# FengDushuo/BBBP-Multi-Modal-Deep-Ensemble-Framework

Measured on AMD Instinct MI355X. Metric: molecules/sec fwd+bwd (3-branch ensemble, B=512), higher is better.
Workload: dtype f32; 1 GPU; MixedInputModel F=167 (MACCS) + 3x128x128 image, 6-layer encoder + 2-stage CNN + fusion + BN head; forward + MSE + backward + fused AdamW, train mode (dropout 0.1); global_batch=512, per_gpu_batch=512, parallelism=dp1, input=device-resident

## Files before the change

bbbp-multi-modal-deep-ensemble-framework_amd/csrc/gemm.hip:

```cpp
#include "common.h"
#include "bbbp_hip.h"
#include <mutex>
#include <type_traits>
#include <unordered_map>

#define TRY_RC(expr) do { int _rc = (expr); if (_rc) return _rc; } while (0)

typedef float f32x4u __attribute__((ext_vector_type(4), aligned(4)));
typedef float f32x2u __attribute__((ext_vector_type(2), aligned(4)));

namespace {

constexpr int bk_of(int tile) { return tile == 64 ? 16 : 32; }

struct GemmParams {
    const float* A; const float* B; float* C;
    const float* bias; const float* R;
    int M, N, K;
    int lda, ldb, ldc, ldr;
    long sA, sB, sC, sR;
    float alpha;
    int act;
    int splits, kchunk;
    float* slab;
// ... 944 lines not shown
    constexpr bool A_KMAJ = (LAYOUT == 2), B_KMAJ = (LAYOUT != 0);
#ifndef BBBP_DIRECT_DEPTH
#define BBBP_DIRECT_DEPTH 4
#endif
    constexpr int D = BBBP_DIRECT_DEPTH;
    const int lane = threadIdx.x & 63, wave = threadIdx.x >> 6;
    const int ks = wave % p.ks, sp = wave / p.ks;
    const int wm = sp / p.wsn, wn = sp % p.wsn;
    DirectOperand<TM, A_KMAJ> opa;
    DirectOperand<TN, B_KMAJ> opb;
    opa.init(p.A + (long)batch * p.sA, p.lda, p.M, (blockIdx.y * p.wsm + wm) * 16 * TM, lane);
    opb.init(p.B + (long)batch * p.sB, p.ldb, p.N, (blockIdx.x * p.wsn + wn) * 16 * TN, lane);

    f32x4 acc[TM][TN];
#pragma unroll
    for (int i = 0; i < TM; ++i)
#pragma unroll
        for (int j = 0; j < TN; ++j) acc[i][j] = f32x4{0.f, 0.f, 0.f, 0.f};
    auto mfma_chunk = [&](const float (&a)[4][TM], const float (&b)[4][TN]) __attribute__((always_inline)) {
#pragma unroll
        for (int j = 0; j < 4; ++j)
#pragma unroll
            for (int um = 0; um < TM; ++um)
#pragma unroll
                for (int un = 0; un < TN; ++un)
                    acc[um][un] = __builtin_amdgcn_mfma_f32_16x16x4f32(a[j][um], b[j][un], acc[um][un], 0, 0, 0);
    };

    const int nch = (p.K + 15) / 16;
    bool has_ones = false;
    if constexpr (LAYOUT == 2) has_ones = p.asum != nullptr && opb.base <= p.N && p.N < opb.base + 16 * TN;
    const int nfast = (nch - 1 > ks) ? (nch - 1 - ks + p.ks - 1) / p.ks : 0;
    if (nfast > 0) {
        float ra[D][4][TM], rb[D][4][TN];
#pragma unroll
        for (int d = 0; d < D; ++d) {
            const int c = ks + min(d, nfast - 1) * p.ks;
            opa.fetch(c, ra[d]); opb.fetch(c, rb[d]);
        }
        for (int i0 = 0; i0 < nfast; i0 += D) {
#pragma unroll
            for (int d = 0; d < D; ++d) {
                if (i0 + d < nfast) {
                    if (has_ones) opb.ones(rb[d], 0, p.K);
                    mfma_chunk(ra[d], rb[d]);
                }
                const int c = ks + min(i0 + d + D, nfast - 1) * p.ks;
                opa.fetch(c, ra[d]); opb.fetch(c, rb[d]);
            }
        }
    }
    if (nch > 0 && (nch - 1) % p.ks == ks) {
        float ta[4][TM], tb[4][TN];
        opa.fetch_tail(nch - 1, p.K, ta); opb.fetch_tail(nch - 1, p.K, tb);
        if (has_ones) opb.ones(tb, nch - 1, p.K);
        mfma_chunk(ta, tb);
    }

    if (p.ks > 1) {
        float* mine = red + (long)wave * (TM * TN * 4 * 64) + lane;
        if (ks != 0) {
#pragma unroll
            for (int um = 0; um < TM; ++um)
#pragma unroll
                for (int un = 0; un < TN; ++un)
#pragma unroll
                    for (int r = 0; r < 4; ++r) mine[((um * TN + un) * 4 + r) * 64] = acc[um][un][r];
        }
        __syncthreads();
        if (ks != 0) return;
        for (int s = 1; s < p.ks; ++s) {
            const float* other = mine + (long)s * (TM * TN * 4 * 64);
#pragma unroll
            for (int um = 0; um < TM; ++um)
#pragma unroll
                for (int un = 0; un < TN; ++un)
#pragma unroll
                    for (int r = 0; r < 4; ++r) acc[um][un][r] += other[((um * TN + un) * 4 + r) * 64];
        }
    }

    float* C = p.C + (long)batch * p.sC;
    const float* R = p.R ? p.R + (long)batch * p.sR : nullptr;
    const int q = lane & 15, kq = lane >> 4;
#pragma unroll
    for (int un = 0; un < TN; ++un) {
        const int n = opb.index(un, q);
        const float bv = (p.bias && n < p.N) ? p.bias[n] : 0.f;
#pragma unroll
        for (int um = 0; um < TM; ++um)
#pragma unroll
            for (int r = 0; r < 4; ++r) {
                const int m = opa.index(um, 4 * kq + r);
                if constexpr (LAYOUT == 2) {
                    if (p.asum && n == p.N && m < p.M) p.asum[(long)batch * p.M + m] = acc[um][un][r];
                }
                if (m < p.M && n < p.N) {
                    float v = apply_act(p.alpha * acc[um][un][r] + bv, p.act);
                    if (p.drop_p > 0.f)
                        v *= dropout_scale(effective_seed(p.drop_seed, p.seed_base), ((uint64_t)batch * p.M + m) * p.N + n, p.drop_p, p.drop_inv_keep);
                    const float gsel = p.gate ? (p.gate[(long)batch * p.sG + (long)m * p.ldg + n] > 0.f ? p.gate_scale : 0.f) : 1.f;
                    if (!p.gate_after) v *= gsel;
                    if (R) v += R[(long)m * p.ldr + n];
                    if (p.gate_after) v *= gsel;
                    C[(long)m * p.ldc + n] = v;
                }
            }
    }
}

template <int LAYOUT, int TM, int TN>
__global__ __launch_bounds__(1024) void gemm_direct_kernel(DirectParams p) {
    BBBP_HIGH_PRIO();
    extern __shared__ float red[];
    gemm_direct_body<LAYOUT, TM, TN>(p, blockIdx.z, red);
}

struct LnFuse {
    const float* gamma; const float* beta;
    float* y; int ldy;
    float* mean; float* rstd;
    float eps;
};

__global__ __launch_bounds__(1024, 2) void gemm_direct_ln_kernel(DirectParams p, LnFuse f) {
    BBBP_HIGH_PRIO();
    __shared__ float part[2][16][16];
    constexpr int D = 4;
    const int lane = threadIdx.x & 63, wave = threadIdx.x >> 6, nw = blockDim.x >> 6;
    const int q = lane & 15, kq = lane >> 4;
    DirectOperand<1, false> opa, opb;
    opa.init(p.A, p.lda, p.M, blockIdx.y * 16, lane);
    opb.init(p.B, p.ldb, p.N, wave * 16, lane);
    f32x4 acc = {0.f, 0.f, 0.f, 0.f};
    auto mfma_chunk = [&](const float (&a)[4][1], const float (&b)[4][1]) __attribute__((always_inline)) {
#pragma unroll
        for (int j = 0; j < 4; ++j) acc = __builtin_amdgcn_mfma_f32_16x16x4f32(a[j][0], b[j][0], acc, 0, 0, 0);
    };
    const int nch = (p.K + 15) / 16;
    const int nfast = nch - 1;
    if (nfast > 0) {
        float ra[D][4][1], rb[D][4][1];
#pragma unroll
        for (int d = 0; d < D; ++d) { const int c = min(d, nfast - 1); opa.fetch(c, ra[d]); opb.fetch(c, rb[d]); }
        for (int i0 = 0; i0 < nfast; i0 += D) {
#pragma unroll
            for (int d = 0; d < D; ++d) {
                if (i0 + d < nfast) mfma_chunk(ra[d], rb[d]);
                const int c = min(i0 + d + D, nfast - 1);
                opa.fetch(c, ra[d]); opb.fetch(c, rb[d]);
            }
        }
    }
    if (nch > 0) {
        float ta[4][1], tb[4][1];
        opa.fetch_tail(nch - 1, p.K, ta); opb.fetch_tail(nch - 1, p.K, tb);
        mfma_chunk(ta, tb);
    }
    const int n = wave * 16 + q, m0 = blockIdx.y * 16 + 4 * kq;
    const bool coln = n < p.N;
    const float bv = (p.bias && coln) ? p.bias[n] : 0.f;
    const uint64_t seed = effective_seed(p.drop_seed, p.seed_base);
    float z[4], s[4];
#pragma unroll
    for (int r = 0; r < 4; ++r) {
        const int m = min(m0 + r, p.M - 1);
        float v = p.alpha * acc[r] + bv;
        if (p.drop_p > 0.f) v *= dropout_scale(seed, (uint64_t)m * p.N + min(n, p.N - 1), p.drop_p, p.drop_inv_keep);
        if (p.R && coln) v += p.R[(long)m * p.ldr + n];
        z[r] = coln ? v : 0.f;
        if (coln && m0 + r < p.M) p.C[(long)m * p.ldc + n] = v;
        s[r] = z[r];
    }
#pragma unroll
    for (int r = 0; r < 4; ++r) { s[r] += __shfl_xor(s[r], 1); s[r] += __shfl_xor(s[r], 2); s[r] += __shfl_xor(s[r], 4); s[r] += __shfl_xor(s[r], 8); }
    if (q == 0) {
#pragma unroll
        for (int r = 0; r < 4; ++r) part[0][wave][4 * kq + r] = s[r];
    }
    __syncthreads();
    float mean[4], d2[4];
#pragma unroll
    for (int r = 0; r < 4; ++r) {
        float t = 0.f;
        for (int w = 0; w < nw; ++w) t += part[0][w][4 * kq + r];
        mean[r] = t / p.N;
        const float d = coln ? z[r] - mean[r] : 0.f;
        d2[r] = d * d;
    }
#pragma unroll
    for (int r = 0; r < 4; ++r) { d2[r] += __shfl_xor(d2[r], 1); d2[r] += __shfl_xor(d2[r], 2); d2[r] += __shfl_xor(d2[r], 4); d2[r] += __shfl_xor(d2[r], 8); }
// ... 574 lines not shown
```

bbbp-multi-modal-deep-ensemble-framework_amd/csrc/rowops.hip:

```cpp
#include "common.h"
#include "bbbp_hip.h"
#include <stdlib.h>
#include <mutex>

namespace {

__device__ __forceinline__ float wave_sum(float v) {
#pragma unroll
    for (int o = 32; o > 0; o >>= 1) v += __shfl_xor(v, o);
    return v;
}
__device__ __forceinline__ float wave_max(float v) {
#pragma unroll
    for (int o = 32; o > 0; o >>= 1) v = fmaxf(v, __shfl_xor(v, o));
    return v;
}

__global__ __launch_bounds__(256) void layernorm_fwd_kernel(float* x, const float* r, float* y, const float* gamma,
                                                           const float* beta, float* mean_out, float* rstd_out,
                                                           int rows, int cols, float eps, float p, uint64_t seed_in, const unsigned long long* seed_base) {
    const uint64_t seed = effective_seed(seed_in, seed_base);
    BBBP_HIGH_PRIO();
    const int lane = threadIdx.x & 63;
    const int row = blockIdx.x * 4 + (threadIdx.x >> 6);
// ... 149 lines not shown
        if (q < nq) {
            const float4 v = make_float4(rs * (g[i].x - s1 - xh[i].x * s2), rs * (g[i].y - s1 - xh[i].y * s2),
                                         rs * (g[i].z - s1 - xh[i].z * s2), rs * (g[i].w - s1 - xh[i].w * s2));
            dzr[q] = v;
            if (dxr) {
                if (p > 0.f) {
                    const float4 k = dropout_scale4(seed, ((uint64_t)row * cols >> 2) + q, p, inv_keep);
                    dxr[q] = make_float4(v.x * k.x, v.y * k.y, v.z * k.z, v.w * k.w);
                } else {
                    dxr[q] = v;
                }
            }
        }
    }
}
inline int ln_wide_nv(int cols) {
    static const int on = bbbp_env_int("BBBP_LN_WIDE", 1);
    return (on && cols >= 1024 && cols <= 4096 && cols % 4 == 0) ? (cols + 1023) / 1024 : 0;
}

constexpr int CW = 16, RL = 32;
__global__ __launch_bounds__(512) void layernorm_param_grad_kernel(const float* dy, const float* z, const float* mean,
                                                                   const float* rstd, float* dgamma, float* dbeta,
                                                                   int rows, int cols) {
    BBBP_HIGH_PRIO();
    __shared__ float s1[RL][CW], s2[RL][CW];
    const int cl = threadIdx.x % CW, rl = threadIdx.x / CW;
    const int c = blockIdx.x * CW + cl;
    float a = 0.f, b = 0.f;
    if (c < cols)
        for (int r = rl; r < rows; r += RL) {
            float g = dy[(long)r * cols + c];
            a += g * (z[(long)r * cols + c] - mean[r]) * rstd[r];
            b += g;
        }
    s1[rl][cl] = a; s2[rl][cl] = b;
    __syncthreads();
    if (rl == 0 && c < cols) {
        float ta = 0.f, tb = 0.f;
#pragma unroll 8
        for (int i = 0; i < RL; ++i) { ta += s1[i][cl]; tb += s2[i][cl]; }
        dgamma[c] = ta; dbeta[c] = tb;
    }
}

__global__ __launch_bounds__(256) void softmax_fwd_kernel(float* x, float* pd, long rows, int cols, float p, uint64_t seed_in, const unsigned long long* seed_base) {
    const uint64_t seed = effective_seed(seed_in, seed_base);
    BBBP_HIGH_PRIO();
    const int lane = threadIdx.x & 63;
    const long row = (long)blockIdx.x * 4 + (threadIdx.x >> 6);
    if (row >= rows) return;
    float* xr = x + row * cols;
    float m = -INFINITY;
    for (int c = lane; c < cols; c += 64) m = fmaxf(m, xr[c]);
    m = wave_max(m);
    float s = 0.f;
    for (int c = lane; c < cols; c += 64) { float e = __expf(xr[c] - m); xr[c] = e; s += e; }
    const float inv = 1.f / wave_sum(s);
    const float inv_keep = p > 0.f ? 1.f / (1.f - p) : 1.f;
    for (int c = lane; c < cols; c += 64) {
        float v = xr[c] * inv;
        xr[c] = v;
        if (pd) pd[row * cols + c] = v * dropout_scale(seed, (uint64_t)row * cols + c, p, inv_keep);
    }
}

__global__ __launch_bounds__(256) void softmax_bwd_kernel(float* dpd, const float* prob, long rows, int cols, float p, uint64_t seed_in, const unsigned long long* seed_base) {
    const uint64_t seed = effective_seed(seed_in, seed_base);
    BBBP_HIGH_PRIO();
    const int lane = threadIdx.x & 63;
    const long row = (long)blockIdx.x * 4 + (threadIdx.x >> 6);
    if (row >= rows) return;
    float* dr = dpd + row * cols;
    const float* pr = prob + row * cols;
    const float inv_keep = p > 0.f ? 1.f / (1.f - p) : 1.f;
    float s = 0.f;
    for (int c = lane; c < cols; c += 64) {
        float d = dr[c];
        if (p > 0.f) { d *= dropout_scale(seed, (uint64_t)row * cols + c, p, inv_keep); dr[c] = d; }
        s += d * pr[c];
    }
    s = wave_sum(s);
    for (int c = lane; c < cols; c += 64) dr[c] = pr[c] * (dr[c] - s);
}

__global__ __launch_bounds__(256) void dropout_kernel(const float* x, float* y, long n, float p, uint64_t seed_in, const unsigned long long* seed_base) {
    const uint64_t seed = effective_seed(seed_in, seed_base);
    BBBP_HIGH_PRIO();
    const float inv_keep = 1.f / (1.f - p);
    for (long i = (long)blockIdx.x * 256 + threadIdx.x; i < n; i += (long)gridDim.x * 256)
        y[i] = x[i] * dropout_scale(seed, (uint64_t)i, p, inv_keep);
}

__global__ __launch_bounds__(1024) void batchnorm_fwd_kernel(const float* x, float* y, const float* gamma, const float* beta,
                                                            float* running_mean, float* running_var, float* save_mean,
                                                            float* save_rstd, int rows, int cols, float eps, float momentum,
                                                            int training) {
    BBBP_HIGH_PRIO();
    __shared__ float red[16][64];
    __shared__ float smean[64], srstd[64];
    const int cl = threadIdx.x & 63, rl = threadIdx.x >> 6;
    const int c = blockIdx.x * 64 + cl;
    if (training) {
        float a = 0.f;
        if (c < cols) for (int r = rl; r < rows; r += 16) a += x[(long)r * cols + c];
        red[rl][cl] = a;
        __syncthreads();
        if (rl == 0) {
            float t = 0.f;
#pragma unroll
            for (int i = 0; i < 16; ++i) t += red[i][cl];
            smean[cl] = t / rows;
        }
        __syncthreads();
        const float mu = smean[cl];
        float q = 0.f;
        if (c < cols) for (int r = rl; r < rows; r += 16) { float d = x[(long)r * cols + c] - mu; q += d * d; }
        __syncthreads();
        red[rl][cl] = q;
        __syncthreads();
        if (rl == 0) {
            float t = 0.f;
#pragma unroll
            for (int i = 0; i < 16; ++i) t += red[i][cl];
            float var = t / rows;
            srstd[cl] = rsqrtf(var + eps);
            if (c < cols) {
                save_mean[c] = mu; save_rstd[c] = srstd[cl];
                running_mean[c] = (1.f - momentum) * running_mean[c] + momentum * mu;
                running_var[c] = (1.f - momentum) * running_var[c] + momentum * var * ((float)rows / (float)(rows - 1));
            }
        }
        __syncthreads();
    } else {
        if (rl == 0 && c < cols) {
            smean[cl] = running_mean[c];
            srstd[cl] = rsqrtf(running_var[c] + eps);
            save_mean[c] = smean[cl]; save_rstd[c] = srstd[cl];
        }
        __syncthreads();
    }
    if (c < cols) {
        const float mu = smean[cl], rs = srstd[cl], g = gamma[c], b = beta[c];
        for (int r = rl; r < rows; r += 16) y[(long)r * cols + c] = (x[(long)r * cols + c] - mu) * rs * g + b;
    }
}

__global__ __launch_bounds__(1024) void batchnorm_bwd_kernel(const float* dy, const float* x, const float* gamma,
                                                            const float* save_mean, const float* save_rstd, float* dx,
                                                            float* dgamma, float* dbeta, int rows, int cols, int training,
                                                            int relu_gate) {
    BBBP_HIGH_PRIO();
    __shared__ float r1[16][64], r2[16][64];
    __shared__ float t1[64], t2[64];
    const int cl = threadIdx.x & 63, rl = threadIdx.x >> 6;
    const int c = blockIdx.x * 64 + cl;
    const float mu = c < cols ? save_mean[c] : 0.f, rs = c < cols ? save_rstd[c] : 0.f;
    float a = 0.f, b = 0.f;
    if (c < cols)
        for (int r = rl; r < rows; r += 16) {
            float g = dy[(long)r * cols + c];
            a += g * (x[(long)r * cols + c] - mu) * rs;
            b += g;
        }
    r1[rl][cl] = a; r2[rl][cl] = b;
    __syncthreads();
// ... 168 lines not shown
}

AdamHyper adam_hyper(double lr, double beta1, double beta2, double eps, double weight_decay, int step, double grad_scale) {
    const double bc1 = 1.0 - pow(beta1, step), bc2 = 1.0 - pow(beta2, step);
    return AdamHyper{(float)(1.0 - lr * weight_decay), (float)(1.0 - beta1), (float)beta2, (float)(1.0 - beta2),
                     (float)(lr / bc1), (float)pow(bc2, 0.5), (float)eps, (float)grad_scale, adamw_background() > 0 ? 1 : 0};
}

__global__ __launch_bounds__(256) void adamw_kernel(float* p, const float* g, float* m, float* v, long n, AdamHyper h) {
    if (!h.low_prio) BBBP_HIGH_PRIO();
    for (long i = (long)blockIdx.x * 256 + threadIdx.x; i < n; i += (long)gridDim.x * 256) {
        float pi = p[i], mi = m[i], vi = v[i];
        adamw_element(pi, g[i], mi, vi, h);
        p[i] = pi; m[i] = mi; v[i] = vi;
    }
}

__global__ void adamw_hyper_store_kernel(float* out, AdamHyper h) {
    if (threadIdx.x == 0) { out[0] = h.decay; out[1] = h.omb1; out[2] = h.beta2; out[3] = h.omb2; out[4] = h.step_size; out[5] = h.bc2_sqrt; out[6] = h.eps; out[7] = h.gscale; }
}

__global__ __launch_bounds__(256) void adamw_multi_kernel(float* __restrict__ p, float* __restrict__ m, float* __restrict__ v, long n,
                                                         const long* __restrict__ offs, const float* const* __restrict__ grads, int nt,
                                                         AdamHyper h, const float* __restrict__ hyper_dev) {
    BBBP_HIGH_PRIO();
    if (hyper_dev) {
        h.decay = hyper_dev[0]; h.omb1 = hyper_dev[1]; h.beta2 = hyper_dev[2]; h.omb2 = hyper_dev[3];
        h.step_size = hyper_dev[4]; h.bc2_sqrt = hyper_dev[5]; h.eps = hyper_dev[6]; h.gscale = hyper_dev[7];
    }
    const long n4 = n & ~3L;
    for (long i = ((long)blockIdx.x * 256 + threadIdx.x) * 4; i < n; i += (long)gridDim.x * 1024) {
        int lo = 0, hi = nt;
        while (hi - lo > 1) { const int mid = (lo + hi) >> 1; if (offs[mid] <= i) lo = mid; else hi = mid; }
        long base = offs[lo], end = offs[lo + 1];
        if (i < n4 && i + 4 <= end) {
            const float* gp = grads[lo] + (i - base);
            float4 pv = *reinterpret_cast<const float4*>(p + i), mv = *reinterpret_cast<const float4*>(m + i), vv = *reinterpret_cast<const float4*>(v + i);
            float g0, g1, g2, g3;
            if ((reinterpret_cast<uintptr_t>(gp) & 15) == 0) { const float4 gv = *reinterpret_cast<const float4*>(gp); g0 = gv.x; g1 = gv.y; g2 = gv.z; g3 = gv.w; }
            else { g0 = gp[0]; g1 = gp[1]; g2 = gp[2]; g3 = gp[3]; }
            adamw_element(pv.x, g0, mv.x, vv.x, h); adamw_element(pv.y, g1, mv.y, vv.y, h);
            adamw_element(pv.z, g2, mv.z, vv.z, h); adamw_element(pv.w, g3, mv.w, vv.w, h);
            *reinterpret_cast<float4*>(p + i) = pv; *reinterpret_cast<float4*>(m + i) = mv; *reinterpret_cast<float4*>(v + i) = vv;
        } else {
            for (long j = i; j < i + 4 && j < n; ++j) {
                while (j >= end) { ++lo; base = offs[lo]; end = offs[lo + 1]; }
                float pj = p[j], mj = m[j], vj = v[j];
                adamw_element(pj, grads[lo][j - base], mj, vj, h);
                p[j] = pj; m[j] = mj; v[j] = vj;
            }
        }
    }
}

__global__ __launch_bounds__(256) void scale_kernel(float* x, long n, float s) {
    BBBP_HIGH_PRIO();
    for (long i = (long)blockIdx.x * 256 + threadIdx.x; i < n; i += (long)gridDim.x * 256) x[i] *= s;
}

inline int grid_for(long n, int background = 0) {
    long g = (n + 255) / 256;
    long cap = background > 0 ? background : (long)bbbp_num_cus() * 8;
    return (int)(g < 1 ? 1 : (g > cap ? cap : g));
}

}

#define ST static_cast<hipStream_t>(stream)

extern "C" int bbbp_layernorm_fwd(void* stream, float* x_inout_z, const float* residual, float* y, const float* gamma,
                                  const float* beta, float* mean, float* rstd, int rows, int cols, float eps,
                                  float dropout_p, uint64_t seed) {
    BBBP_CHECK_ARG(rows >= 0 && cols > 0, "layernorm: bad shape %d x %d", rows, cols);
    BBBP_CHECK_ARG(dropout_p >= 0.f && dropout_p < 1.f, "layernorm: bad dropout %f", dropout_p);
    if (rows == 0) return BBBP_OK;
#define BBBP_LN_FWD_WIDE(NV) hipLaunchKernelGGL(layernorm_fwd_wide_kernel<NV>, dim3(rows), dim3(256), g_bbbp_small_lds_pad, ST, x_inout_z, residual, \
                                                y, gamma, beta, mean, rstd, rows, cols, eps, dropout_p, seed, g_bbbp_seed_base)
    switch (ln_wide_nv(cols)) {
        case 1: BBBP_LN_FWD_WIDE(1); break;
        case 2: BBBP_LN_FWD_WIDE(2); break;
        case 3: BBBP_LN_FWD_WIDE(3); break;
        case 4: BBBP_LN_FWD_WIDE(4); break;
        default:
            hipLaunchKernelGGL(layernorm_fwd_kernel, dim3(cdiv(rows, 4)), dim3(256), g_bbbp_small_lds_pad, ST, x_inout_z, residual, y, gamma, beta,
                               mean, rstd, rows, cols, eps, dropout_p, seed, g_bbbp_seed_base);
    }
#undef BBBP_LN_FWD_WIDE
    BBBP_CHECK_LAUNCH();
    return BBBP_OK;
}

extern "C" int bbbp_layernorm_bwd(void* stream, const float* dy, const float* z, const float* gamma, const float* mean,
                                  const float* rstd, float* dz, float* dx, float* dgamma, float* dbeta, int rows, int cols,
                                  float dropout_p, uint64_t seed) {
    BBBP_CHECK_ARG(rows >= 0 && cols > 0, "layernorm bwd: bad shape %d x %d", rows, cols);
    if (rows > 0 && dz) {
#define BBBP_LN_BWD_WIDE(NV) hipLaunchKernelGGL(layernorm_bwd_wide_kernel<NV>, dim3(rows), dim3(256), g_bbbp_small_lds_pad, ST, dy, z, gamma, mean, \
                                                rstd, dz, dx, rows, cols, dropout_p, seed, g_bbbp_seed_base)
        switch (ln_wide_nv(cols)) {
            case 1: BBBP_LN_BWD_WIDE(1); break;
            case 2: BBBP_LN_BWD_WIDE(2); break;
            case 3: BBBP_LN_BWD_WIDE(3); break;
            case 4: BBBP_LN_BWD_WIDE(4); break;
            default:
                hipLaunchKernelGGL(layernorm_bwd_kernel, dim3(cdiv(rows, 4)), dim3(256), g_bbbp_small_lds_pad, ST, dy, z, gamma, mean, rstd, dz, dx,
                                   rows, cols, dropout_p, seed, g_bbbp_seed_base);
        }
#undef BBBP_LN_BWD_WIDE
        BBBP_CHECK_LAUNCH();
    }
    if (dgamma) {
        hipLaunchKernelGGL(layernorm_param_grad_kernel, dim3(cdiv(cols, CW)), dim3(CW * RL), g_bbbp_small_lds_pad, ST, dy, z, mean, rstd, dgamma,
                           dbeta, rows, cols);
        BBBP_CHECK_LAUNCH();
    }
    return BBBP_OK;
}

extern "C" int bbbp_softmax_fwd(void* stream, float* x_inout, float* dropped_out, long rows, int cols, float dropout_p,
                                uint64_t seed) {
    BBBP_CHECK_ARG(rows >= 0 && cols > 0, "softmax: bad shape");
    if (rows == 0) return BBBP_OK;
    hipLaunchKernelGGL(softmax_fwd_kernel, dim3((unsigned)((rows + 3) / 4)), dim3(256), g_bbbp_small_lds_pad, ST, x_inout,
                       dropout_p > 0.f ? dropped_out : nullptr, rows, cols, dropout_p, seed, g_bbbp_seed_base);
    BBBP_CHECK_LAUNCH();
    return BBBP_OK;
}

extern "C" int bbbp_softmax_bwd(void* stream, float* dprob_inout, const float* prob, long rows, int cols, float dropout_p,
                                uint64_t seed) {
    BBBP_CHECK_ARG(rows >= 0 && cols > 0, "softmax bwd: bad shape");
    if (rows == 0) return BBBP_OK;
    hipLaunchKernelGGL(softmax_bwd_kernel, dim3((unsigned)((rows + 3) / 4)), dim3(256), g_bbbp_small_lds_pad, ST, dprob_inout, prob, rows, cols,
                       dropout_p, seed, g_bbbp_seed_base);
    BBBP_CHECK_LAUNCH();
    return BBBP_OK;
}

extern "C" int bbbp_dropout(void* stream, const float* x, float* y, long n, float p, uint64_t seed) {
    BBBP_CHECK_ARG(p >= 0.f && p < 1.f, "dropout: bad p %f", p);
    if (n == 0) return BBBP_OK;
    if (p == 0.f) {
        if (x != y) BBBP_CHECK_HIP(hipMemcpyAsync(y, x, n * sizeof(float), hipMemcpyDeviceToDevice, ST));
        return BBBP_OK;
    }
    hipLaunchKernelGGL(dropout_kernel, dim3(grid_for(n)), dim3(256), g_bbbp_small_lds_pad, ST, x, y, n, p, seed, g_bbbp_seed_base);
    BBBP_CHECK_LAUNCH();
    return BBBP_OK;
}

extern "C" int bbbp_batchnorm1d_fwd(void* stream, const float* x, float* y, const float* gamma, const float* beta,
                                    float* running_mean, float* running_var, float* save_mean, float* save_rstd, int rows,
                                    int cols, float eps, float momentum, int training) {
    BBBP_CHECK_ARG(cols > 0 && rows >= 0, "batchnorm: bad shape");
    BBBP_CHECK_ARG(!(training && rows <= 1), "Expected more than 1 value per channel when training, got input size [%d, %d]", rows, cols);
    if (rows == 0) return BBBP_OK;
    hipLaunchKernelGGL(batchnorm_fwd_kernel, dim3(cdiv(cols, 64)), dim3(1024), g_bbbp_small_lds_pad, ST, x, y, gamma, beta, running_mean,
                       running_var, save_mean, save_rstd, rows, cols, eps, momentum, training);
    BBBP_CHECK_LAUNCH();
    return BBBP_OK;
}

extern "C" int bbbp_batchnorm1d_bwd(void* stream, const float* dy, const float* x, const float* gamma, const float* save_mean,
                                    const float* save_rstd, float* dx, float* dgamma, float* dbeta, int rows, int cols,
                                    int training) {
    BBBP_CHECK_ARG(cols > 0 && rows >= 0, "batchnorm bwd: bad shape");
    hipLaunchKernelGGL(batchnorm_bwd_kernel, dim3(cdiv(cols, 64)), dim3(1024), g_bbbp_small_lds_pad, ST, dy, x, gamma, save_mean, save_rstd, dx,
                       dgamma, dbeta, rows, cols, training, 0);
    BBBP_CHECK_LAUNCH();
    return BBBP_OK;
}

extern "C" int bbbp_batchnorm1d_bwd_relu(void* stream, const float* dy, const float* x, const float* gamma, const float* save_mean,
                                         const float* save_rstd, float* dx, float* dgamma, float* dbeta, int rows, int cols,
                                         int training) {
    BBBP_CHECK_ARG(cols > 0 && rows >= 0, "batchnorm bwd: bad shape");
    hipLaunchKernelGGL(batchnorm_bwd_kernel, dim3(cdiv(cols, 64)), dim3(1024), g_bbbp_small_lds_pad, ST, dy, x, gamma, save_mean, save_rstd, dx,
                       dgamma, dbeta, rows, cols, training, 1);
    BBBP_CHECK_LAUNCH();
    return BBBP_OK;
}

extern "C" int bbbp_column_moments(void* stream, const float* x, const float* centre, float* sum_out, float* sumsq_out, int rows,
                                   int cols) {
    BBBP_CHECK_ARG(rows >= 0 && cols > 0 && x && sum_out && sumsq_out, "column_moments: bad arguments");
    hipLaunchKernelGGL(column_moments_kernel, dim3(cdiv(cols, 16)), dim3(512), g_bbbp_small_lds_pad, ST, x, centre, sum_out, sumsq_out,
                       rows, cols);
    BBBP_CHECK_LAUNCH();
    return BBBP_OK;
}

extern "C" int bbbp_batchnorm1d_bwd_apply(void* stream, const float* dy, const float* x, const float* gamma, const float* mean,
                                          const float* rstd, const float* sum_dy, const float* sum_dy_xhat, float* dx, int rows,
                                          int cols, long n_global) {
    BBBP_CHECK_ARG(rows >= 0 && cols > 0 && n_global >= 1, "batchnorm bwd_apply: bad arguments");
    if (rows == 0) return BBBP_OK;
    long total = (long)rows * cols;
    hipLaunchKernelGGL(batchnorm_bwd_apply_kernel, dim3(grid_for(total)), dim3(256), g_bbbp_small_lds_pad, ST, dy, x, gamma, mean, rstd,
                       sum_dy, sum_dy_xhat, dx, total, cols, 1.0f / (float)n_global);
    BBBP_CHECK_LAUNCH();
    return BBBP_OK;
}

extern "C" int bbbp_bias_act_bwd(void* stream, float* dy_inout, int lddy, const float* y, int ldy, float* dbias, int rows,
                                 int cols, int act, float scale) {
    BBBP_CHECK_ARG(cols > 0 && rows >= 0 && act >= 0 && act <= 2, "bias_act_bwd: bad args");
    BBBP_CHECK_ARG(act == 0 || y, "bias_act_bwd: activation output required");
    hipLaunchKernelGGL(bias_act_bwd_kernel, dim3(cdiv(cols, CW)), dim3(CW * RL), g_bbbp_small_lds_pad, ST, dy_inout, lddy, y, ldy, dbias, rows, cols,
                       act, scale);
    BBBP_CHECK_LAUNCH();
    return BBBP_OK;
}

extern "C" int bbbp_fusion_combine_fwd(void* stream, const float* combined, const float* hid, const float* const* w2,
                                       const float* const* b2, float* out, float* attn, int rows, int dim, int hidden,
                                       int num_heads) {
    BBBP_CHECK_ARG(num_heads >= 1 && num_heads <= 8, "fusion: num_heads %d not in [1, 8]", num_heads);
// ... 152 lines not shown
```

Baseline: 211,200 molecules/s.

## Register-resident row kernels for LN/softmax and batched loads in GEMM epilogue

Adds templated layernorm and softmax forward/backward kernels that keep a whole row in registers, sized by column count. They issue all global loads up front with clamped indices, under a waves-per-EU budget and scheduling barriers, instead of re-reading the row in strided loops. The direct GEMM epilogue is restructured to gather bias, gate and residual values up front with clamped indices, compute all outputs, then store them, so loads overlap rather than serialize per element. This adds template instantiations and register pressure, and relies on inline-asm pins and scheduling barriers that could constrain the compiler.

New measurement: 211,700 molecules/s (median of 6 runs). About the same (+0.3%).

```diff
diff --git a/bbbp-multi-modal-deep-ensemble-framework_amd/csrc/gemm.hip b/bbbp-multi-modal-deep-ensemble-framework_amd/csrc/gemm.hip
--- a/bbbp-multi-modal-deep-ensemble-framework_amd/csrc/gemm.hip
+++ b/bbbp-multi-modal-deep-ensemble-framework_amd/csrc/gemm.hip
@@ -1050,31 +1050,71 @@
 
     float* C = p.C + (long)batch * p.sC;
     const float* R = p.R ? p.R + (long)batch * p.sR : nullptr;
-    const int q = lane & 15, kq = lane >> 4;
-#pragma unroll
-    for (int un = 0; un < TN; ++un) {
-        const int n = opb.index(un, q);
-        const float bv = (p.bias && n < p.N) ? p.bias[n] : 0.f;
+    const float* G = p.gate ? p.gate + (long)batch * p.sG : nullptr;
+    int lane_e = lane;
+    asm volatile("" : "+v"(lane_e));
+    const int q = lane_e & 15, kq = lane_e >> 4;
+    int nn[TN], nc[TN], mm[TM][4], mc[TM][4];
+    float bv[TN], gv[TN][TM][4], rv[TN][TM][4], out[TN][TM][4];
+#pragma unroll
+    for (int un = 0; un < TN; ++un) { nn[un] = opb.index(un, q); nc[un] = min(nn[un], p.N - 1); }
+#pragma unroll
+    for (int um = 0; um < TM; ++um)
+#pragma unroll
+        for (int r = 0; r < 4; ++r) { mm[um][r] = opa.index(um, 4 * kq + r); mc[um][r] = min(mm[um][r], p.M - 1); }
+#pragma unroll
+    for (int un = 0; un < TN; ++un) bv[un] = p.bias ? p.bias[nc[un]] : 0.f;
+    if (G) {
+#pragma unroll
+        for (int un = 0; un < TN; ++un)
+#pragma unroll
+            for (int um = 0; um < TM; ++um)
+#pragma unroll
+                for (int r = 0; r < 4; ++r) gv[un][um][r] = G[(long)mc[um][r] * p.ldg + nc[un]];
+    }
+    if (R) {
+#pragma unroll
+        for (int un = 0; un < TN; ++un)
+#pragma unroll
+            for (int um = 0; um < TM; ++um)
+#pragma unroll
+                for (int r = 0; r < 4; ++r) rv[un][um][r] = R[(long)mc[um][r] * p.ldr + nc[un]];
+    }
+#pragma unroll
+    for (int un = 0; un < TN; ++un)
 #pragma unroll
         for (int um = 0; um < TM; ++um)
 #pragma unroll
             for (int r = 0; r < 4; ++r) {
-                const int m = opa.index(um, 4 * kq + r);
+                const int m = mm[um][r], n = nn[un];
+                float v = apply_act(p.alpha * acc[um][un][r] + bv[un], p.act);
+                if (p.drop_p > 0.f)
+                    v *= dropout_scale(effective_seed(p.drop_seed, p.seed_base), ((uint64_t)batch * p.M + m) * p.N + n, p.drop_p, p.drop_inv_keep);
+                const float gsel = G ? (gv[un][um][r] > 0.f ? p.gate_scale : 0.f) : 1.f;
+                if (!p.gate_after) v *= gsel;
+                if (R) v += rv[un][um][r];
+                if (p.gate_after) v *= gsel;
+                out[un][um][r] = v;
+                __builtin_amdgcn_sched_barrier(0);
+            }
+#pragma unroll
+    for (int un = 0; un < TN; ++un)
+#pragma unroll
+        for (int um = 0; um < TM; ++um)
+#pragma unroll
+            for (int r = 0; r < 4; ++r) asm volatile("" : "+v"(out[un][um][r]));
+#pragma unroll
+    for (int un = 0; un < TN; ++un)
+#pragma unroll
+        for (int um = 0; um < TM; ++um)
+#pragma unroll
+            for (int r = 0; r < 4; ++r) {
+                const int m = mm[um][r], n = nn[un];
                 if constexpr (LAYOUT == 2) {
                     if (p.asum && n == p.N && m < p.M) p.asum[(long)batch * p.M + m] = acc[um][un][r];
                 }
-                if (m < p.M && n < p.N) {
-                    float v = apply_act(p.alpha * acc[um][un][r] + bv, p.act);
-                    if (p.drop_p > 0.f)
-                        v *= dropout_scale(effective_seed(p.drop_seed, p.seed_base), ((uint64_t)batch * p.M + m) * p.N + n, p.drop_p, p.drop_inv_keep);
-                    const float gsel = p.gate ? (p.gate[(long)batch * p.sG + (long)m * p.ldg + n] > 0.f ? p.gate_scale : 0.f) : 1.f;
-                    if (!p.gate_after) v *= gsel;
-                    if (R) v += R[(long)m * p.ldr + n];
-                    if (p.gate_after) v *= gsel;
-                    C[(long)m * p.ldc + n] = v;
-                }
-            }
-    }
+                if (m < p.M && n < p.N) C[(long)m * p.ldc + n] = out[un][um][r];
+            }
 }
 
 template <int LAYOUT, int TM, int TN>
diff --git a/bbbp-multi-modal-deep-ensemble-framework_amd/csrc/rowops.hip b/bbbp-multi-modal-deep-ensemble-framework_amd/csrc/rowops.hip
--- a/bbbp-multi-modal-deep-ensemble-framework_amd/csrc/rowops.hip
+++ b/bbbp-multi-modal-deep-ensemble-framework_amd/csrc/rowops.hip
@@ -255,6 +255,206 @@
     }
     s = wave_sum(s);
     for (int c = lane; c < cols; c += 64) dr[c] = pr[c] * (dr[c] - s);
+}
+
+#define BBBP_PIN(x) asm volatile("" : "+v"(x))
+
+#define BBBP_ROW_REG_BUDGET __attribute__((amdgpu_waves_per_eu(8)))
+template <int NV>
+__global__ __launch_bounds__(256) BBBP_ROW_REG_BUDGET void layernorm_fwd_reg_kernel(float* x, const float* r, float* y, const float* gamma,
+                                                               const float* beta, float* mean_out, float* rstd_out,
+                                                               int rows, int cols, float eps, float p, uint64_t seed_in, const unsigned long long* seed_base) {
+    const uint64_t seed = effective_seed(seed_in, seed_base);
+    BBBP_HIGH_PRIO();
+    __builtin_assume(cols > 0 && cols <= 64 * NV);
+    const int lane = threadIdx.x & 63;
+    const int row = blockIdx.x * 4 + __builtin_amdgcn_readfirstlane(threadIdx.x >> 6);
+    if (row >= rows) return;
+    float* xr = x + (long)row * cols;
+    const float* rr = r ? r + (long)row * cols : nullptr;
+    float* yr = y + (long)row * cols;
+    const float inv_keep = p > 0.f ? 1.f / (1.f - p) : 1.f;
+    float v[NV], a[NV], g[NV], b[NV];
+#pragma unroll
+    for (int i = 0; i < NV; ++i) {
+        const unsigned cc = min(lane + 64 * i, cols - 1);
+        v[i] = xr[cc]; g[i] = gamma[cc]; b[i] = beta[cc];
+        a[i] = rr ? rr[cc] : 0.f;
+    }
+    __builtin_amdgcn_sched_barrier(0);
+    float s = 0.f;
+#pragma unroll
+    for (int i = 0; i < NV; ++i) {
+        const unsigned c = lane + 64 * i;
+        if (c < (unsigned)cols) {
+            if (p > 0.f) v[i] *= dropout_scale(seed, (uint64_t)row * cols + c, p, inv_keep);
+            if (rr) v[i] += a[i];
+            s += v[i];
+        }
+        __builtin_amdgcn_sched_barrier(0);
+    }
+    const float mean = wave_sum(s) / cols;
+    float q = 0.f;
+#pragma unroll
+    for (int i = 0; i < NV; ++i)
+        if (lane + 64 * i < cols) { float d = v[i] - mean; q += d * d; }
+    const float rstd = rsqrtf(wave_sum(q) / cols + eps);
+    float o[NV];
+#pragma unroll
+    for (int i = 0; i < NV; ++i) { o[i] = (v[i] - mean) * rstd * g[i] + b[i]; BBBP_PIN(o[i]); }
+#pragma unroll
+    for (int i = 0; i < NV; ++i) {
+        const unsigned c = lane + 64 * i;
+        if (c < (unsigned)cols) { xr[c] = v[i]; yr[c] = o[i]; }
+    }
+    if (lane == 0) { mean_out[row] = mean; rstd_out[row] = rstd; }
+}
+
+template <int NV>
+__global__ __launch_bounds__(256) BBBP_ROW_REG_BUDGET void layernorm_bwd_reg_kernel(const float* dy, const float* z, const float* gamma,
+                                                               const float* mean, const float* rstd, float* dz, float* dx,
+                                                               int rows, int cols, float p, uint64_t seed_in, const unsigned long long* seed_base) {
+#pragma clang fp contract(off)
+    const uint64_t seed = effective_seed(seed_in, seed_base);
+    BBBP_HIGH_PRIO();
+    __builtin_assume(cols > 0 && cols <= 64 * NV);
+    const int lane = threadIdx.x & 63;
+    const int row = blockIdx.x * 4 + __builtin_amdgcn_readfirstlane(threadIdx.x >> 6);
+    if (row >= rows) return;
+    const float* dyr = dy + (long)row * cols;
+    const float* zr = z + (long)row * cols;
+    const float mu = mean[row], rs = rstd[row];
+    float d[NV], zz[NV], w[NV];
+#pragma unroll
+    for (int i = 0; i < NV; ++i) {
+        const unsigned cc = min(lane + 64 * i, cols - 1);
+        d[i] = dyr[cc]; w[i] = gamma[cc]; zz[i] = zr[cc];
+    }
+    __builtin_amdgcn_sched_barrier(0);
+    float s1 = 0.f, s2 = 0.f;
+#pragma unroll
+    for (int i = 0; i < NV; ++i) {
+        if (lane + 64 * i < cols) {
+            const float g = d[i] * w[i];
+            s1 += g;
+            s2 += g * (zz[i] - mu) * rs;
+        }
+    }
+    s1 = wave_sum(s1) / cols;
+    s2 = wave_sum(s2) / cols;
+    const float inv_keep = p > 0.f ? 1.f / (1.f - p) : 1.f;
+    float o[NV], od[NV];
+#pragma unroll
+    for (int i = 0; i < NV; ++i) {
+        const unsigned c = lane + 64 * i;
+        const float vv = rs * fmaf(-s2, (zz[i] - mu) * rs, fmaf(d[i], w[i], -s1));
+        o[i] = vv;
+        od[i] = (dx && p > 0.f) ? vv * dropout_scale(seed, (uint64_t)row * cols + min(c, (unsigned)cols - 1), p, inv_keep) : vv;
+        BBBP_PIN(o[i]); BBBP_PIN(od[i]);
+        __builtin_amdgcn_sched_barrier(0);
+    }
+#pragma unroll
+    for (int i = 0; i < NV; ++i) {
+        const unsigned c = lane + 64 * i;
+        if (c < (unsigned)cols) {
+            dz[(long)row * cols + c] = o[i];
+            if (dx) dx[(long)row * cols + c] = od[i];
+        }
+    }
+}
+
+template <int NV>
+__global__ __launch_bounds__(256) BBBP_ROW_REG_BUDGET void softmax_fwd_reg_kernel(float* x, float* pd, long rows, int cols, float p, uint64_t seed_in, const unsigned long long* seed_base) {
+    const uint64_t seed = effective_seed(seed_in, seed_base);
+    BBBP_HIGH_PRIO();
+    __builtin_assume(cols > 0 && cols <= 64 * NV);
+    const int lane = threadIdx.x & 63;
+    const long row = (long)blockIdx.x * 4 + __builtin_amdgcn_readfirstlane(threadIdx.x >> 6);
+    if (row >= rows) return;
+    float* xr = x + row * cols;
+    float v[NV];
+#pragma unroll
+    for (int i = 0; i < NV; ++i) v[i] = xr[(unsigned)min(lane + 64 * i, cols - 1)];
+    __builtin_amdgcn_sched_barrier(0);
+    float m = -INFINITY;
+#pragma unroll
+    for (int i = 0; i < NV; ++i)
+        if (lane + 64 * i < cols) m = fmaxf(m, v[i]);
+    m = wave_max(m);
+    float s = 0.f;
+#pragma unroll
+    for (int i = 0; i < NV; ++i)
+        if (lane + 64 * i < cols) { float e = __expf(v[i] - m); v[i] = e; s += e; }
+    const float inv = 1.f / wave_sum(s);
+    const float inv_keep = p > 0.f ? 1.f / (1.f - p) : 1.f;
+#pragma unroll
+    for (int i = 0; i < NV; ++i) {
+        const unsigned c = lane + 64 * i;
+        if (c < (unsigned)cols) {
+            float val = v[i] * inv;
+            xr[c] = val;
+            if (pd) pd[row * cols + c] = val * dropout_scale(seed, (uint64_t)row * cols + c, p, inv_keep);
+        }
+        __builtin_amdgcn_sched_barrier(0);
+    }
+}
+
+template <int NV>
+__global__ __launch_bounds__(256) BBBP_ROW_REG_BUDGET void softmax_bwd_reg_kernel(float* dpd, const float* prob, long rows, int cols, float p, uint64_t seed_in, const unsigned long long* seed_base) {
+    const uint64_t seed = effective_seed(seed_in, seed_base);
+    BBBP_HIGH_PRIO();
+    __builtin_assume(cols > 0 && cols <= 64 * NV);
+    const int lane = threadIdx.x & 63;
+    const long row = (long)blockIdx.x * 4 + __builtin_amdgcn_readfirstlane(threadIdx.x >> 6);
+    if (row >= rows) return;
+    float* dr = dpd + row * cols;
+    const float* pr = prob + row * cols;
+    const float inv_keep = p > 0.f ? 1.f / (1.f - p) : 1.f;
+    constexpr bool EARLY = NV > 12;
+    unsigned keep = 0;
+    if (EARLY && p > 0.f) {
+#pragma unroll
+        for (int i = 0; i < NV; ++i) {
+            const unsigned c = lane + 64 * i;
+            if (c < (unsigned)cols) keep |= (dropout_scale(seed, (uint64_t)row * cols + c, p, inv_keep) != 0.f ? 1u : 0u) << i;
+            __builtin_amdgcn_sched_barrier(0);
+        }
+    }
+    float d[NV], pv[NV];
+#pragma unroll
+    for (int i = 0; i < NV; ++i) {
+        const unsigned cc = min(lane + 64 * i, cols - 1);
+        d[i] = dr[cc]; pv[i] = pr[cc];
+    }
+    __builtin_amdgcn_sched_barrier(0);
+    float s = 0.f;
+#pragma unroll
+    for (int i = 0; i < NV; ++i) {
+        const unsigned c = lane + 64 * i;
+        if (c < (unsigned)cols) {
+            if (p > 0.f) d[i] *= EARLY ? ((keep >> i) & 1u ? inv_keep : 0.f) : dropout_scale(seed, (uint64_t)row * cols + c, p, inv_keep);
+            s += d[i] * pv[i];
+        }
+        __builtin_amdgcn_sched_barrier(0);
+    }
+    s = wave_sum(s);
+#pragma unroll
+    for (int i = 0; i < NV; ++i) { d[i] = pv[i] * (d[i] - s); BBBP_PIN(d[i]); }
+#pragma unroll
+    for (int i = 0; i < NV; ++i) {
+        const unsigned c = lane + 64 * i;
+        if (c < (unsigned)cols) dr[c] = d[i];
+    }
+}
+#undef BBBP_PIN
+#undef BBBP_ROW_REG_BUDGET
+
+inline int row_reg_nv(int cols, int max_nv) {
+    const int nv = (cols + 63) / 64;
+    if (nv > max_nv) return 0;
+    for (int b : {1, 2, 3, 4, 6, 8, 12, 16})
+        if (nv <= b) return b;
+    return 0;
 }
 
 __global__ __launch_bounds__(256) void dropout_kernel(const float* x, float* y, long n, float p, uint64_t seed_in, const unsigned long long* seed_base) {
@@ -589,8 +789,20 @@
         case 3: BBBP_LN_FWD_WIDE(3); break;
         case 4: BBBP_LN_FWD_WIDE(4); break;
         default:
-            hipLaunchKernelGGL(layernorm_fwd_kernel, dim3(cdiv(rows, 4)), dim3(256), g_bbbp_small_lds_pad, ST, x_inout_z, residual, y, gamma, beta,
-                               mean, rstd, rows, cols, eps, dropout_p, seed, g_bbbp_seed_base);
+#define BBBP_LN_FWD_REG(NV) hipLaunchKernelGGL(layernorm_fwd_reg_kernel<NV>, dim3(cdiv(rows, 4)), dim3(256), g_bbbp_small_lds_pad, ST, x_inout_z, \
+                                               residual, y, gamma, beta, mean, rstd, rows, cols, eps, dropout_p, seed, g_bbbp_seed_base)
+            switch (row_reg_nv(cols, 8)) {
+                case 1: BBBP_LN_FWD_REG(1); break;
+                case 2: BBBP_LN_FWD_REG(2); break;
+                case 3: BBBP_LN_FWD_REG(3); break;
+                case 4: BBBP_LN_FWD_REG(4); break;
+                case 6: BBBP_LN_FWD_REG(6); break;
+                case 8: BBBP_LN_FWD_REG(8); break;
+                default:
+                    hipLaunchKernelGGL(layernorm_fwd_kernel, dim3(cdiv(rows, 4)), dim3(256), g_bbbp_small_lds_pad, ST, x_inout_z, residual, y, gamma,
+                                       beta, mean, rstd, rows, cols, eps, dropout_p, seed, g_bbbp_seed_base);
+            }
+#undef BBBP_LN_FWD_REG
     }
 #undef BBBP_LN_FWD_WIDE
     BBBP_CHECK_LAUNCH();
@@ -610,8 +822,20 @@
             case 3: BBBP_LN_BWD_WIDE(3); break;
             case 4: BBBP_LN_BWD_WIDE(4); break;
             default:
-                hipLaunchKernelGGL(layernorm_bwd_kernel, dim3(cdiv(rows, 4)), dim3(256), g_bbbp_small_lds_pad, ST, dy, z, gamma, mean, rstd, dz, dx,
-                                   rows, cols, dropout_p, seed, g_bbbp_seed_base);
+#define BBBP_LN_BWD_REG(NV) hipLaunchKernelGGL(layernorm_bwd_reg_kernel<NV>, dim3(cdiv(rows, 4)), dim3(256), g_bbbp_small_lds_pad, ST, dy, z, gamma, \
+                                               mean, rstd, dz, dx, rows, cols, dropout_p, seed, g_bbbp_seed_base)
+                switch (row_reg_nv(cols, 8)) {
+                    case 1: BBBP_LN_BWD_REG(1); break;
+                    case 2: BBBP_LN_BWD_REG(2); break;
+                    case 3: BBBP_LN_BWD_REG(3); break;
+                    case 4: BBBP_LN_BWD_REG(4); break;
+                    case 6: BBBP_LN_BWD_REG(6); break;
+                    case 8: BBBP_LN_BWD_REG(8); break;
+                    default:
+                        hipLaunchKernelGGL(layernorm_bwd_kernel, dim3(cdiv(rows, 4)), dim3(256), g_bbbp_small_lds_pad, ST, dy, z, gamma, mean, rstd, dz,
+                                           dx, rows, cols, dropout_p, seed, g_bbbp_seed_base);
+                }
+#undef BBBP_LN_BWD_REG
         }
 #undef BBBP_LN_BWD_WIDE
         BBBP_CHECK_LAUNCH();
@@ -628,8 +852,20 @@
                                 uint64_t seed) {
     BBBP_CHECK_ARG(rows >= 0 && cols > 0, "softmax: bad shape");
     if (rows == 0) return BBBP_OK;
-    hipLaunchKernelGGL(softmax_fwd_kernel, dim3((unsigned)((rows + 3) / 4)), dim3(256), g_bbbp_small_lds_pad, ST, x_inout,
-                       dropout_p > 0.f ? dropped_out : nullptr, rows, cols, dropout_p, seed, g_bbbp_seed_base);
+#define BBBP_SM_FWD(K) hipLaunchKernelGGL(K, dim3((unsigned)((rows + 3) / 4)), dim3(256), g_bbbp_small_lds_pad, ST, x_inout, \
+                                          dropout_p > 0.f ? dropped_out : nullptr, rows, cols, dropout_p, seed, g_bbbp_seed_base)
+    switch (row_reg_nv(cols, 16)) {
+        case 1: BBBP_SM_FWD(softmax_fwd_reg_kernel<1>); break;
+        case 2: BBBP_SM_FWD(softmax_fwd_reg_kernel<2>); break;
+        case 3: BBBP_SM_FWD(softmax_fwd_reg_kernel<3>); break;
+        case 4: BBBP_SM_FWD(softmax_fwd_reg_kernel<4>); break;
+        case 6: BBBP_SM_FWD(softmax_fwd_reg_kernel<6>); break;
+        case 8: BBBP_SM_FWD(softmax_fwd_reg_kernel<8>); break;
+        case 12: BBBP_SM_FWD(softmax_fwd_reg_kernel<12>); break;
+        case 16: BBBP_SM_FWD(softmax_fwd_reg_kernel<16>); break;
+        default: BBBP_SM_FWD(softmax_fwd_kernel);
+    }
+#undef BBBP_SM_FWD
     BBBP_CHECK_LAUNCH();
     return BBBP_OK;
 }
@@ -638,8 +874,20 @@
                                 uint64_t seed) {
     BBBP_CHECK_ARG(rows >= 0 && cols > 0, "softmax bwd: bad shape");
     if (rows == 0) return BBBP_OK;
-    hipLaunchKernelGGL(softmax_bwd_kernel, dim3((unsigned)((rows + 3) / 4)), dim3(256), g_bbbp_small_lds_pad, ST, dprob_inout, prob, rows, cols,
-                       dropout_p, seed, g_bbbp_seed_base);
+#define BBBP_SM_BWD(K) hipLaunchKernelGGL(K, dim3((unsigned)((rows + 3) / 4)), dim3(256), g_bbbp_small_lds_pad, ST, dprob_inout, prob, rows, cols, \
+                                          dropout_p, seed, g_bbbp_seed_base)
+    switch (row_reg_nv(cols, 16)) {
+        case 1: BBBP_SM_BWD(softmax_bwd_reg_kernel<1>); break;
+        case 2: BBBP_SM_BWD(softmax_bwd_reg_kernel<2>); break;
+        case 3: BBBP_SM_BWD(softmax_bwd_reg_kernel<3>); break;
+        case 4: BBBP_SM_BWD(softmax_bwd_reg_kernel<4>); break;
+        case 6: BBBP_SM_BWD(softmax_bwd_reg_kernel<6>); break;
+        case 8: BBBP_SM_BWD(softmax_bwd_reg_kernel<8>); break;
+        case 12: BBBP_SM_BWD(softmax_bwd_reg_kernel<12>); break;
+        case 16: BBBP_SM_BWD(softmax_bwd_reg_kernel<16>); break;
+        default: BBBP_SM_BWD(softmax_bwd_kernel);
+    }
+#undef BBBP_SM_BWD
     BBBP_CHECK_LAUNCH();
     return BBBP_OK;
 }
```
